# divideon/xvc

Measured on AMD Instinct MI355X. Metric: hot-path frame passes/s (TZ + sub-pel ME, MC, transform + RDOQ + dequant + inverse, deblock, pad, PSNR parts), bit-exact vs the reference's classes, higher is better.
Workload: dtype u16; 1 GPU; 1920x1080 yuv420p 30fps synthetic, QP 32, internal bitdepth 10, 16x16 CUs, TZ range 96, RDOQ (RdoQuant::QuantRdo + CoeffSignHideRdo, picture-initial CABAC contexts); cus_per_picture=8160, parallelism=3 independent picture chains in flight

## Files before the change

### xvc_amd/csrc/k_recon.h

```cpp
#ifndef XVCGPU_K_RECON_H_
#define XVCGPU_K_RECON_H_

#include <stddef.h>

#include <type_traits>

#include "dev_common.h"
#include "dev_tables.h"
#include "k_me2.h"
#include "k_tx2.h"
#include "xvcgpu_internal.h"

struct __attribute__((aligned(16))) ReconShared {
  Tx2Shared tx;
  uint16_t pred[256];
  int16_t tmp[16 * 23];
  uint16_t win[23 * 24];
};

template <bool CHROMA, int FW = 0, int FH = 0>
__device__ __forceinline__ void wave_interp_block_lds(int bd, int w_in, int h_in, int fx, int fy,
                                                      const uint16_t *ref, int rs,
                                                      uint16_t *win, int16_t *tmp,
                                                      uint16_t *dst) {
// ... 66 lines not shown
  hpass(std::true_type());
  wave_sync();
  {
    const int sh2 = 6 + (14 - bd);
    const int off2 = (8192 << 6) + (1 << (sh2 - 1));
    lane_loop<NS, 64>(lane, w * h, [&](int i) {
      const int16_t *s = tmp + i;
      int sum = 0;
#pragma unroll
      for (int k = 0; k < N; k++) sum += (int)s[k * w] * fv[k];
      dst[i] = d_clip_bd((int16_t)((sum + off2) >> sh2), smax);
    });
  }
}

template <bool RDOQ, bool FWD>
__device__ __forceinline__ void recon_from_me_kernel_body(PicView orig, PicView ref, PicView rec, const xvcgpu_me_block *blocks, const xvcgpu_me_result *results, int n_cus, int qp_y, int qp_c, int intra_pic, int ref_poc, int32_t *nnz_out, xvcgpu_cu_info *cus, const int16_t *tx_tables, const int16_t *tx_tables_t, TxTableLayout lay, const xvcgpu_rdoq_contexts *rq_ctx, const xvcgpu_rdoq_params *rq_prm, int16_t *coeffs, const uint32_t *coeff_off, FwdClassify fc) {
  constexpr int TXM = FWD ? TX_MODE_FWD : TX_MODE_FULL;
  __shared__ ReconShared s_all[4];
  union RqWave {
    RdoqShared<256> one;
    RdoqShared<64> two[2];
  };
  __shared__ RqWave rq_all[RDOQ ? 4 : 1];
  RdoqShared<256> *rq_wave = &rq_all[RDOQ ? (threadIdx.x >> 6) : 0].one;
  ReconShared &s = s_all[threadIdx.x >> 6];
  FwdClassify fcl = fc;
  if constexpr (FWD) {
    __shared__ RqProveLds pv_all[4];
    fcl.pv = (fc.cls && fc.rq_ctx && fc.rq_prm) ? &pv_all[threadIdx.x >> 6] : nullptr;
    if (fcl.pv && (threadIdx.x & 63) == 0) fcl.pv->staged_ctx = -1;
  }
  const int n = n_cus * 2;
  const int n_wg = (n + 3) / 4;
  const int wg = xcd_job_index(blockIdx.x, n_wg);
  if (wg < 0) return;
  const int job = __builtin_amdgcn_readfirstlane(wg * 4 + (int)(threadIdx.x >> 6));
  if (job >= n) return;
  const int ci = job >> 1;
  const bool chroma = (job & 1) != 0;
#ifdef XVCGPU_TRACE
  const int bi = job;
#endif
  ME2_TRACE(0);
  static_assert(offsetof(xvcgpu_me_block, y) == 2 && offsetof(xvcgpu_me_block, w) == 4 &&
                    offsetof(xvcgpu_me_block, h) == 5 && alignof(xvcgpu_me_block) >= 4,
                "xvcgpu_me_block: x, y, w, h in its first two dwords");
  const uint32_t *mbq = reinterpret_cast<const uint32_t *>(blocks + ci);
  const uint32_t mb0 = mbq[0], mb1 = mbq[1];
  const struct {
    int x, y, w, h;
  } mb = {(int16_t)(mb0 & 0xffff), (int16_t)(mb0 >> 16), (int)(mb1 & 0xff), (int)((mb1 >> 8) & 0xff)};
  const xvcgpu_me_result mr = results[ci];
  const int bd = ref.bd;
  int mx = mr.mv_x, my = mr.mv_y;
  d_clip_mv(mb.x, mb.y, ref.c[0].w, ref.c[0].h, mx, my);
  const bool cu16 = __builtin_expect(mb.w == 16 && mb.h == 16, 1);
  xvcgpu_tx_block tb;
  tb.tx_hor = XVC_TX_DEFAULT;
  tb.tx_ver = XVC_TX_DEFAULT;
  tb.dst4x4 = 0;
  tb.intra_pic = (uint8_t)intra_pic;
  if (chroma) {
    auto cjob = [&](auto exact) __attribute__((always_inline)) {
      constexpr int FS = decltype(exact)::value ? 8 : 0;
      constexpr int shift = 5;
      const int fx = mx & 31, fy = my & 31;
      const int cx = mb.x >> 1, cy = mb.y >> 1;
      const int cw = FS ? FS : mb.w >> 1, ch = FS ? FS : mb.h >> 1;
      const int lw = 31 - __clz(cw);
      tb.x = (int16_t)cx;
      tb.y = (int16_t)cy;
      tb.w = (uint8_t)cw;
      tb.h = (uint8_t)ch;
      const int g = ME2_LANE >> 5, comp = 1 + g;
      const PlaneView po = g ? orig.c[2] : orig.c[1];
      const PlaneView pc = g ? rec.c[2] : rec.c[1];
      const int i4 = (ME2_LANE & 31) * 4;
      const bool mine = i4 < cw * ch;
      U16x4 orig_pre = {{0u, 0u}};
      if (mine)
        orig_pre = *reinterpret_cast<const U16x4 *>(
            po.p + (ptrdiff_t)(cy + (i4 >> lw)) * po.stride + cx + (i4 & (cw - 1)));
#pragma unroll
      for (int c = 1; c <= 2; c++) {
        const PlaneView prf = ref.c[c];
        const uint16_t *r =
            prf.p + (ptrdiff_t)(cy + (my >> shift)) * prf.stride + cx + (mx >> shift);
        wave_interp_block_lds<true, FS, FS>(bd, cw, ch, fx, fy, r, prf.stride, s.win, s.tmp,
                                            s.pred + (c - 1) * 64);
        wave_sync();
      }
      ME2_TRACE(1);
      tb.comp = (uint8_t)comp;
      tb.qp = (int8_t)qp_c;
      if (FWD && mine)
        *reinterpret_cast<U16x4 *>(pc.p + (ptrdiff_t)(cy + (i4 >> lw)) * pc.stride + cx +
                                   (i4 & (cw - 1))) =
            *reinterpret_cast<const U16x4 *>(s.pred + g * 64 + i4);
      tx2_job<TXM, 32, RDOQ, FS, FS>(
          s.tx, tb, 3 * ci + comp, bd, po, s.pred + g * 64, cw, pc, FWD ? coeffs : nullptr,
          FWD ? coeff_off : nullptr, nnz_out, tx_tables, tx_tables_t, lay, &orig_pre, g * 128,
          reinterpret_cast<RdoqShared<64> *>(rq_wave) + g, rq_ctx, rq_prm, nullptr,
          FWD ? &fcl : nullptr);
      ME2_TRACE(8);
    };
    if (cu16) cjob(std::true_type());
    else cjob(std::false_type());
    return;
  }
  auto ljob = [&](auto exact) __attribute__((always_inline)) {
    constexpr int FS = decltype(exact)::value ? 16 : 0;
    constexpr int shift = 4;
    const int fx = mx & 15, fy = my & 15;
    const int cx = mb.x, cy = mb.y;
    const int cw = FS ? FS : mb.w, ch = FS ? FS : mb.h;
    const int lw = 31 - __clz(cw);
    tb.x = (int16_t)cx;
    tb.y = (int16_t)cy;
    tb.w = (uint8_t)cw;
    tb.h = (uint8_t)ch;
    const PlaneView prf = ref.c[0];
    const uint16_t *r = prf.p + (ptrdiff_t)(cy + (my >> shift)) * prf.stride + cx + (mx >> shift);
    U16x4 orig_pre = {{0u, 0u}};
    {
      const int i = ME2_LANE * 4;
      if (i < cw * ch) {
        const PlaneView po = orig.c[0];
        orig_pre = *reinterpret_cast<const U16x4 *>(
            po.p + (ptrdiff_t)(cy + (i >> lw)) * po.stride + cx + (i & (cw - 1)));
      }
    }
    wave_interp_block_lds<false, FS, FS>(bd, cw, ch, fx, fy, r, prf.stride, s.win, s.tmp, s.pred);
    wave_sync();
    ME2_TRACE(1);
    tb.comp = 0;
    tb.qp = (int8_t)qp_y;
    if (FWD) {
      const PlaneView pc = rec.c[0];
      lane_loop<FS * FS, 256>(ME2_LANE * 4, cw * ch, [&](int i) {
        *reinterpret_cast<U16x4 *>(pc.p + (ptrdiff_t)(cy + (i >> lw)) * pc.stride + cx +
                                   (i & (cw - 1))) = *reinterpret_cast<const U16x4 *>(s.pred + i);
      });
    }
    const int nnz = tx2_job<TXM, 64, RDOQ, FS, FS>(s.tx, tb, 3 * ci, bd, orig.c[0], s.pred, cw, rec.c[0],
                                         FWD ? coeffs : nullptr, FWD ? coeff_off : nullptr,
                                         nnz_out, tx_tables, tx_tables_t, lay, &orig_pre, 0,
                                         rq_wave, rq_ctx, rq_prm, nullptr, FWD ? &fcl : nullptr);
    ME2_TRACE(8);
    if (cus && ME2_LANE == 0) {
      xvcgpu_cu_info c;
      c.x = (uint16_t)mb.x;
      c.y = (uint16_t)mb.y;
      c.w = (uint8_t)cw;
      c.h = (uint8_t)ch;
      c.intra = 0;
      c.cbf_luma = !FWD && nnz != 0;
      c.qp_y = (int8_t)qp_y;
      c.qp_c = (int8_t)qp_c;
      c.ref_idx0 = 0;
      c.reserved = 0;
      c.ref_poc[0] = ref_poc;
      c.ref_poc[1] = -1;
      for (int k = 0; k < 4; k++) {
        c.mv[0][k][0] = mr.mv_x;
        c.mv[0][k][1] = mr.mv_y;
        c.mv[1][k][0] = 0;
        c.mv[1][k][1] = 0;
      }
      cus[ci] = c;
    }
  };
  if (cu16) ljob(std::true_type());
  else ljob(std::false_type());
}

#ifndef RECON_FWD_MIN_WAVES
#define RECON_FWD_MIN_WAVES 7
#endif
template <bool RDOQ = false, bool FWD = false>
__global__ void __launch_bounds__(256, FWD && !RDOQ ? RECON_FWD_MIN_WAVES : 1)
recon_from_me_kernel(PicView orig, PicView ref, PicView rec, const xvcgpu_me_block *blocks, const xvcgpu_me_result *results, int n_cus, int qp_y, int qp_c, int intra_pic, int ref_poc, int32_t *nnz_out, xvcgpu_cu_info *cus, const int16_t *tx_tables, const int16_t *tx_tables_t, TxTableLayout lay, const xvcgpu_rdoq_contexts *rq_ctx = nullptr, const xvcgpu_rdoq_params *rq_prm = nullptr, int16_t *coeffs = nullptr, const uint32_t *coeff_off = nullptr, FwdClassify fc = FwdClassify()) {
  recon_from_me_kernel_body<RDOQ, FWD>(orig, ref, rec, blocks, results, n_cus, qp_y, qp_c, intra_pic, ref_poc, nnz_out, cus, tx_tables, tx_tables_t, lay, rq_ctx, rq_prm, coeffs, coeff_off, fc);
}

#endif
```

### xvc_amd/csrc/k_tx2.h

```cpp
#ifndef XVCGPU_K_TX2_H_
#define XVCGPU_K_TX2_H_

#include "dev_common.h"
#include "dev_tables.h"
#include "k_me.h"
#include "k_me2.h"
#include "k_tx.h"
#include "xvcgpu_internal.h"

#define TX2_WAVES 4

typedef short tx2_v2s __attribute__((ext_vector_type(2)));

struct __attribute__((aligned(16))) Tx2Shared {
  int16_t r[256];
  int16_t t[256];
  int16_t c[256];
};

__device__ __forceinline__ int tx2_dot2(uint32_t a, uint32_t b, int acc) {
  return __builtin_amdgcn_sdot2(__builtin_bit_cast(tx2_v2s, a),
                                __builtin_bit_cast(tx2_v2s, b), acc, false);
}

template <int NJ>
__device__ __forceinline__ void tx2_load_row(const int16_t *p, uint32_t *d) {
  if (NJ == 4) {
    const uint2 v = *reinterpret_cast<const uint2 *>(p);
    d[0] = v.x; d[1] = v.y;
  } else {
#pragma unroll
    for (int q = 0; q < NJ / 8; q++) {
      const uint4 v = *reinterpret_cast<const uint4 *>(p + 8 * q);
      d[4 * q] = v.x; d[4 * q + 1] = v.y; d[4 * q + 2] = v.z; d[4 * q + 3] = v.w;
    }
  }
}

template <int NJ, int OPL, bool CLIP, int G = 64>
__device__ __forceinline__ void tx2_stage(const int16_t *A, const int16_t *B,
                                          int na, int nb, int add, int shift,
                                          int16_t *out) {
  const int lane = ME2_LANE & (G - 1);
  const int gb = nb / OPL;
  const int a = lane >> (31 - __clz(gb)), b0 = (lane & (gb - 1)) * OPL;
  if (a >= na) return;
  uint32_t ra[NJ / 2];
  tx2_load_row<NJ>(A + a * NJ, ra);
  int16_t res[OPL];
#pragma unroll
  for (int o = 0; o < OPL; o++) {
    uint32_t rb[NJ / 2];
    tx2_load_row<NJ>(B + (b0 + o) * NJ, rb);
    int acc = add;
#pragma unroll
    for (int j = 0; j < NJ / 2; j++) acc = tx2_dot2(ra[j], rb[j], acc);
    int v = acc >> shift;
    if (CLIP) v = d_clip3(v, -32768, 32767);
    res[o] = (int16_t)v;
  }
  int16_t *dst = out + a * nb + b0;
  if (OPL == 4) {
    *reinterpret_cast<uint2 *>(dst) =
        make_uint2((uint16_t)res[0] | ((uint32_t)(uint16_t)res[1] << 16),
                   (uint16_t)res[2 % OPL] | ((uint32_t)(uint16_t)res[3 % OPL] << 16));
  } else if (OPL == 2) {
    *reinterpret_cast<uint32_t *>(dst) =
        (uint16_t)res[0] | ((uint32_t)(uint16_t)res[1 % OPL] << 16);
  } else {
    dst[0] = res[0];
  }
}

template <bool CLIP, int G = 64>
__device__ __forceinline__ void tx2_stage_dispatch(int nj, const int16_t *A,
                                                   const int16_t *B, int na, int nb,
                                                   int add, int shift, int16_t *out) {
  const int total = na * nb;
  if (nj == 16) {
    if (total > 2 * G) tx2_stage<16, 4, CLIP, G>(A, B, na, nb, add, shift, out);
    else if (total > G) tx2_stage<16, 2, CLIP, G>(A, B, na, nb, add, shift, out);
    else tx2_stage<16, 1, CLIP, G>(A, B, na, nb, add, shift, out);
  } else if (nj == 8) {
    if (total > 2 * G) tx2_stage<8, 4, CLIP, G>(A, B, na, nb, add, shift, out);
    else if (total > G) tx2_stage<8, 2, CLIP, G>(A, B, na, nb, add, shift, out);
    else tx2_stage<8, 1, CLIP, G>(A, B, na, nb, add, shift, out);
  } else {
    if (total > 2 * G) tx2_stage<4, 4, CLIP, G>(A, B, na, nb, add, shift, out);
    else if (total > G) tx2_stage<4, 2, CLIP, G>(A, B, na, nb, add, shift, out);
    else tx2_stage<4, 1, CLIP, G>(A, B, na, nb, add, shift, out);
  }
}

template <int G>
__device__ __forceinline__ int tx2_group_add(int v) {
  if (G == 64) return wave_reduce_add_i32(v);
  v = dpp_group_sum<16>(v);
  return v + __shfl_xor(v, 16, 64);
}

struct FwdClassify {
  signed char *cls;
  int16_t *levels;
  int32_t *nnz;
  const xvcgpu_rdoq_contexts *rq_ctx;
  const xvcgpu_rdoq_params *rq_prm;
  RqProveLds *pv;
};

template <int MODE, int G = 64, bool RDOQ = false, int FW = 0, int FH = 0>
__device__ __forceinline__ int tx2_job(Tx2Shared &sh, const xvcgpu_tx_block &b, int bi,
                                       int bd, const PlaneView &po, const uint16_t *pred_p,
                                       int pred_stride, const PlaneView &pr,
                                       int16_t *levels, const uint32_t *level_off,
                                       int32_t *nnz_out, const int16_t *tx_tables,
                                       const int16_t *tx_tables_t,
                                       const TxTableLayout &lay,
                                       const U16x4 *orig_pre = nullptr, int soff = 0,
                                       RdoqShared<(G == 32 ? 64 : 256)> *rq = nullptr,
                                       const xvcgpu_rdoq_contexts *rq_ctx = nullptr,
                                       const xvcgpu_rdoq_params *rq_prm = nullptr,
                                       unsigned long long *dist_out = nullptr,
                                       const FwdClassify *fc = nullptr) {
  struct { int16_t *r, *t, *c; } s = {sh.r + soff, sh.t + soff, sh.c + soff};
  unsigned long long dist_acc = 0;
  auto dist4 = [&](int y, int x, const U16x4 &p, int r0, int r1, int r2, int r3) {
    const U16x4 o = *reinterpret_cast<const U16x4 *>(po.p + (ptrdiff_t)(b.y + y) * po.stride +
                                                     b.x + x);
    const int d0 = (int)(o.v[0] & 0xffff) - (int)(p.v[0] & 0xffff) - r0;
    const int d1 = (int)(o.v[0] >> 16) - (int)(p.v[0] >> 16) - r1;
    const int d2 = (int)(o.v[1] & 0xffff) - (int)(p.v[1] & 0xffff) - r2;
    const int d3 = (int)(o.v[1] >> 16) - (int)(p.v[1] >> 16) - r3;
    dist_acc += (unsigned long long)((long long)d0 * d0) + (unsigned long long)((long long)d1 * d1) +
                (unsigned long long)((long long)d2 * d2) + (unsigned long long)((long long)d3 * d3);
  };
  auto dist_finish = [&]() {
    unsigned long long v = dist_acc;
#pragma unroll
    for (int sft = 1; sft < G; sft <<= 1) v += __shfl_xor(v, sft, 64);
    if ((ME2_LANE & (G - 1)) == 0) dist_out[bi] = v >> (2 * (bd - 8));
  };
  const int lane = ME2_LANE & (G - 1);
  const int w = FW ? FW : b.w, h = FH ? FH : b.h;
  const int lw = 31 - __clz(w);
  const int lgw = lw, lgh = 31 - __clz(h);
  int16_t *lv = (levels && level_off) ? levels + level_off[bi] : nullptr;
  const int offh = tx_table_off(lay, b.tx_hor, w), offv = tx_table_off(lay, b.tx_ver, h);
  const int16_t *Mh = tx_tables + offh, *Mv = tx_tables + offv;
  const int16_t *MhT = tx_tables_t + offh, *MvT = tx_tables_t + offv;

  int qpb = b.qp + 6 * (bd - 8);
  qpb = qpb > 0 ? qpb : 0;
  const bool bias = ((lgw + lgh) & 1) != 0;
  const int tshift = 15 - bd - ((lgw + lgh) >> 1);
  const int n_el = w * h;
  constexpr int NE = FW * FH;

  int nnz;
  if (MODE != TX_MODE_INV) {
    lane_loop<NE, 4 * G>(lane * 4, n_el, [&](int i) {
      const int y = i >> lw, x = i & (w - 1);
      const U16x4 o = orig_pre ? *orig_pre
                               : *reinterpret_cast<const U16x4 *>(
                                     po.p + (ptrdiff_t)(b.y + y) * po.stride + b.x + x);
      const U16x4 p = *reinterpret_cast<const U16x4 *>(
          pred_p + (ptrdiff_t)y * pred_stride + x);
      const int d0 = (int)(o.v[0] & 0xffff) - (int)(p.v[0] & 0xffff);
      const int d1 = (int)(o.v[0] >> 16) - (int)(p.v[0] >> 16);
      const int d2 = (int)(o.v[1] & 0xffff) - (int)(p.v[1] & 0xffff);
      const int d3 = (int)(o.v[1] >> 16) - (int)(p.v[1] >> 16);
      *reinterpret_cast<uint2 *>(s.r + i) =
          make_uint2((uint32_t)(d0 & 0xffff) | ((uint32_t)d1 << 16),
                     (uint32_t)(d2 & 0xffff) | ((uint32_t)d3 << 16));
    });
    wave_sync();
    ME2_TRACE(2);
    const int shift1 = lgw + bd - 9 + (b.tx_hor == XVC_TX_DCT2_LOW ? 0 : 2);
    const int shift2 = lgh + 6 + (b.tx_ver == XVC_TX_DCT2_LOW ? 0 : 2);
    tx2_stage_dispatch<false, G>(w, Mh, s.r, w, h, 1 << (shift1 - 1), shift1, s.t);
    wave_sync();
    ME2_TRACE(3);
    tx2_stage_dispatch<false, G>(h, s.t, Mv, w, h, 1 << (shift2 - 1), shift2, s.c);
    wave_sync();
    ME2_TRACE(4);
    if (MODE == TX_MODE_FWD) {
      if (fc && fc->cls) {
        const int fq_shift = 14 + qpb / 6 + tshift + (bias ? 7 : 0);
        const int fq_scale = kFwdQuantScales[qpb % 6] * (bias ? 181 : 1);
        const long long fq_offset = 1ll << (fq_shift - 1);
        bool any = false;
        RqProveLds *pv = fc->pv;
        const int grp = ME2_LANE / G;
        if (pv) {
          if (lane == 0) {
            pv->n[grp] = 0;
            pv->fail[grp] = 0;
          }
          wave_sync();
        }
        lane_loop<NE, G>(lane, n_el, [&](int i) {
          const int a = (short)d_abs((int)s.c[i]);
          const bool nz = (short)(int)((((long long)a * fq_scale) + fq_offset) >> fq_shift) != 0;
          any |= nz;
          if (pv && nz) {
            const int slot = atomicAdd(&pv->n[grp], 1);
            if (slot < RQ_PROVE_MAX_CANDS)
              pv->xy[grp][slot] = (unsigned short)(((i & (h - 1)) << 8) | (i >> lgh));
            if (a < 0) pv->fail[grp] = 1;
          }
        });
        const unsigned long long group =
            G == 64 ? ~0ull : (((1ull << G) - 1) << (ME2_LANE & ~(G - 1)));
        bool live = (__ballot(any) & group) != 0;
        if (pv) {
          wave_sync();
          if (rq_prove_zero_lds<G>(*pv, b, bd, fc->rq_ctx, fc->rq_prm[bi], s.c, live)) live = false;
        }
        if (lane == 0) fc->cls[bi] = live ? (signed char)rq_class_of(b) : (signed char)-1;
        if (!live) {
          int16_t *z = fc->levels + level_off[bi];
          lane_loop<NE, G>(lane, n_el, [&](int i) { z[i] = 0; });
          if (lane == 0 && fc->nnz) fc->nnz[bi] = 0;
          return 0;
        }
      }
      if (lv)
        lane_loop<NE, G>(lane, n_el, [&](int i) {
          const int x = i >> lgh, k2 = i & (h - 1);
          lv[k2 * w + x] = s.c[i];
        });
      return 0;
    }
    const bool intra_pic = (b.intra_pic & XVC_TXF_INTRA_PIC) != 0;
    const bool sign_hide = !(b.intra_pic & XVC_TXF_NO_SIGN_HIDING);
    const int scan_order = (b.intra_pic >> XVC_TXF_SCAN_SHIFT) & 3;
    const int qshift = 14 + qpb / 6 + tshift + (bias ? 7 : 0);
    const int qscale = kFwdQuantScales[qpb % 6] * (bias ? 181 : 1);
    const long long qoff = (long long)((intra_pic ? 171ull : 85ull) << (qshift - 9));
    const bool use_rdoq = RDOQ && (b.intra_pic & XVC_TXF_RDOQ) != 0;
    if (RDOQ && use_rdoq) {
      const xvcgpu_rdoq_params prm = rq_prm[bi];
      const int16_t *cfp = s.c;
      int16_t *lvp = s.r;
      auto cf_at = [cfp, h](int x, int y) { return (int)cfp[x * h + y]; };
      auto lv_at = [lvp, h](int x, int y) { return lvp + x * h + y; };
      if (G == 64 && rq4_takes(64, w, h, scan_order)) {
        rq_stage_costs(&rq_ctx[prm.ctx_index], rq->ctx_bits, lane, 64);
        wave_sync();
        nnz = wave_rdoq4<64, 1>(*rq, lane, bd, w, h, b.qp, b.comp == 0, sign_hide, prm, cf_at,
                                lv_at);
      } else {
        nnz = wave_rdoq<G>(*rq, lane, bd, w, h, b.qp, b.comp == 0, scan_order, sign_hide,
                           rq_ctx[prm.ctx_index], prm, cf_at, lv_at);
      }
      wave_sync();
    }
    int local = 0;
    if (!use_rdoq) {
    for (int i = lane; i < n_el; i += G) {
      const int v = s.c[i];
      const int sign = v < 0 ? -1 : 1;
      const long long abs_coeff = d_abs(v);
      const int level = (int)(((abs_coeff * qscale) + qoff) >> qshift);
      local += level != 0;
      s.r[i] = (int16_t)d_clip3(level * sign, -32768, 32767);
      s.t[i] = (int16_t)(((abs_coeff * qscale) - ((long long)level << qshift)) >> (qshift - 8));
    }
    nnz = tx2_group_add<G>(local);
    }
    if (!use_rdoq && sign_hide && nnz > 1 && w >= 4 && h >= 4) {
      wave_sync();
      const int gw = w >> 2, gh = h >> 2;
      auto idx = [h](int x, int y) { return x * h + y; };
      const bool mine = lane < gw * gh;
      const int sx = mine ? (lane & (gw - 1)) : 0, sy = mine ? (lane >> (lgw - 2)) : 0;
      bool any = false;
      if (mine)
        for (int k = 0; k < 16; k++) any |= s.r[idx(4 * sx + (k & 3), 4 * sy + (k >> 2))] != 0;
      const int my_scan = d_sb_scan_index(scan_order, gw, gh, sx, sy);
      int last_sb = any ? my_scan : -1;
#pragma unroll
      for (int sft = 1; sft < 16; sft <<= 1) {
        const int o = __shfl_xor(last_sb, sft, 64);
// ... 73 lines not shown
      if (dist_out) dist4(y, x, p, cf, cf, cf, cf);
    });
    if (dist_out) dist_finish();
    return nnz;
  }
  {
    const int shift1 = 7 + (b.tx_ver == XVC_TX_DCT2_LOW ? 0 : 2);
    const int shift2 = 20 - bd + (b.tx_hor == XVC_TX_DCT2_LOW ? 0 : 2);
    tx2_stage_dispatch<true, G>(h, MvT, s.c, h, w, 1 << (shift1 - 1), shift1, s.r);
    wave_sync();
    tx2_stage_dispatch<true, G>(w, s.r, MhT, h, w, 1 << (shift2 - 1), shift2, s.t);
    wave_sync();
    ME2_TRACE(7);
  }
  lane_loop<NE, 4 * G>(lane * 4, n_el, [&](int i) {
    const int y = i >> lw, x = i & (w - 1);
    const U16x4 p = *reinterpret_cast<const U16x4 *>(
        pred_p + (ptrdiff_t)y * pred_stride + x);
    const uint2 rs = *reinterpret_cast<const uint2 *>(s.t + i);
    U16x4 o;
    o.v[0] = (uint32_t)d_clip3((int)(p.v[0] & 0xffff) + (int)(int16_t)(rs.x & 0xffff), 0, smax) |
             ((uint32_t)d_clip3((int)(p.v[0] >> 16) + ((int)rs.x >> 16), 0, smax) << 16);
    o.v[1] = (uint32_t)d_clip3((int)(p.v[1] & 0xffff) + (int)(int16_t)(rs.y & 0xffff), 0, smax) |
             ((uint32_t)d_clip3((int)(p.v[1] >> 16) + ((int)rs.y >> 16), 0, smax) << 16);
    *reinterpret_cast<U16x4 *>(pr.p + (ptrdiff_t)(b.y + y) * pr.stride + b.x + x) = o;
    if (dist_out)
      dist4(y, x, p, (int)(int16_t)(rs.x & 0xffff), (int)rs.x >> 16, (int)(int16_t)(rs.y & 0xffff),
            (int)rs.y >> 16);
  });
  if (dist_out) dist_finish();
  return nnz;
}

template <int MODE, bool RDOQ>
__device__ __forceinline__ void residual_wave_kernel_body(PicView orig, PicView pred, PicView rec, const xvcgpu_tx_block *blocks, int n, int16_t *levels, const uint32_t *level_off, int32_t *nnz_out, const int16_t *tx_tables, const int16_t *tx_tables_t, TxTableLayout lay, const xvcgpu_rdoq_contexts *rq_ctx, const xvcgpu_rdoq_params *rq_prm, unsigned long long *dist_out) {
  __shared__ Tx2Shared s_all[TX2_WAVES];
  __shared__ RdoqShared<256> rq_all[RDOQ ? TX2_WAVES : 1];
  Tx2Shared &s = s_all[threadIdx.x >> 6];
  const int n_wg = (n + TX2_WAVES - 1) / TX2_WAVES;
  const int wg = xcd_job_index(blockIdx.x, n_wg);
  if (wg < 0) return;
  const int bi = __builtin_amdgcn_readfirstlane(wg * TX2_WAVES + (int)(threadIdx.x >> 6));
  if (bi >= n) return;
  if (MODE == TX_MODE_INV && !dist_out && pred.c[0].p == rec.c[0].p && nnz_out[bi] == 0) return;
  const xvcgpu_tx_block b = blocks[bi];
  if (!tx_small_job(b)) return;
  const PlaneView pp = pred.c[b.comp];
  tx2_job<MODE, 64, RDOQ>(s, b, bi, pred.bd, orig.c[b.comp],
                          pp.p + (ptrdiff_t)b.y * pp.stride + b.x, pp.stride, rec.c[b.comp],
                          levels, level_off, nnz_out, tx_tables, tx_tables_t, lay, nullptr, 0,
                          &rq_all[RDOQ ? (threadIdx.x >> 6) : 0], rq_ctx, rq_prm, dist_out);
}

__global__ void __launch_bounds__(64 * TX2_WAVES)
inv_cu_pairs_kernel(PicView rec, const xvcgpu_tx_block *blocks, int n_cus, int16_t *levels,
                    const uint32_t *level_off, int32_t *nnz_out, const int16_t *tx_tables,
                    const int16_t *tx_tables_t, TxTableLayout lay) {
  const int n = 2 * n_cus;
  const int n_wg = (n + TX2_WAVES - 1) / TX2_WAVES;
  const int wg = xcd_job_index(blockIdx.x, n_wg);
  if (wg < 0) return;
  const int job = __builtin_amdgcn_readfirstlane(wg * TX2_WAVES + (int)(threadIdx.x >> 6));
  if (job >= n) return;
  const int ci = job >> 1;
  if (!(job & 1)) {
    if (nnz_out[3 * ci] == 0) return;
  } else {
    if (nnz_out[3 * ci + 1] == 0 && nnz_out[3 * ci + 2] == 0) return;
  }
  __shared__ Tx2Shared s_all[TX2_WAVES];
  Tx2Shared &s = s_all[threadIdx.x >> 6];
  if (!(job & 1)) {
    const int bi = 3 * ci;
    const xvcgpu_tx_block b = blocks[bi];
    if (!tx_small_job(b)) return;
    const PlaneView pc = rec.c[0];
    const uint16_t *at = pc.p + (ptrdiff_t)b.y * pc.stride + b.x;
    if (__builtin_expect(b.w == 16 && b.h == 16, 1))
      tx2_job<TX_MODE_INV, 64, false, 16, 16>(s, b, bi, rec.bd, pc, at, pc.stride, pc, levels,
                                              level_off, nnz_out, tx_tables, tx_tables_t, lay);
    else
      tx2_job<TX_MODE_INV, 64, false>(s, b, bi, rec.bd, pc, at, pc.stride, pc, levels, level_off,
                                      nnz_out, tx_tables, tx_tables_t, lay);
    return;
  }
  const int g = ME2_LANE >> 5, bi = 3 * ci + 1 + g;
  const xvcgpu_tx_block b = blocks[bi];
  if (!tx_small_job(b) || b.w * b.h > 64) return;
  const PlaneView pc = g ? rec.c[2] : rec.c[1];
  const uint16_t *at = pc.p + (ptrdiff_t)b.y * pc.stride + b.x;
  if (__builtin_expect(b.w == 8 && b.h == 8, 1))
    tx2_job<TX_MODE_INV, 32, false, 8, 8>(s, b, bi, rec.bd, pc, at, pc.stride, pc, levels,
                                          level_off, nnz_out, tx_tables, tx_tables_t, lay,
                                          nullptr, g * 128);
  else
    tx2_job<TX_MODE_INV, 32, false>(s, b, bi, rec.bd, pc, at, pc.stride, pc, levels, level_off,
                                    nnz_out, tx_tables, tx_tables_t, lay, nullptr, g * 128);
}

template <int MODE, bool RDOQ = false>
__global__ void __launch_bounds__(64 * TX2_WAVES)
residual_wave_kernel(PicView orig, PicView pred, PicView rec, const xvcgpu_tx_block *blocks, int n, int16_t *levels, const uint32_t *level_off, int32_t *nnz_out, const int16_t *tx_tables, const int16_t *tx_tables_t, TxTableLayout lay, const xvcgpu_rdoq_contexts *rq_ctx = nullptr, const xvcgpu_rdoq_params *rq_prm = nullptr, unsigned long long *dist_out = nullptr) {
  residual_wave_kernel_body<MODE, RDOQ>(orig, pred, rec, blocks, n, levels, level_off, nnz_out, tx_tables, tx_tables_t, lay, rq_ctx, rq_prm, dist_out);
}

template <int MODE, bool RDOQ>
__device__ __forceinline__ void
residual_cu_body(const PicView &orig, const PicView &pred, const PicView &rec, const xvcgpu_tx_block *blocks, int n,
                   int16_t *levels, const uint32_t *level_off, int32_t *nnz_out,
                   const int16_t *tx_tables, const int16_t *tx_tables_t, TxTableLayout lay,
                   const xvcgpu_rdoq_contexts *rq_ctx, const xvcgpu_rdoq_params *rq_prm,
                   const xvcgpu_block_pos *src_pos, const xvcgpu_eval_cand *ecands, int n_head,
                   uint64_t *eout, int strength) {
  struct Big {
    TxShared s;
    RdoqShared<RDOQ ? 1024 : 4> rq;
  };
  struct Small {
    Tx2Shared s;
    RdoqShared<256> rq;
  };
  constexpr size_t kBytes = sizeof(Big) > sizeof(Small) ? sizeof(Big) : sizeof(Small);
  __shared__ __attribute__((aligned(16))) unsigned char raw[kBytes];
  const int idx = blockIdx.x;
  auto price = [&](int c) {
    const xvcgpu_eval_cand cd = ecands[c];
    const PlaneView pa = orig.c[cd.comp], pb = cd.versus ? rec.c[cd.comp] : pred.c[cd.comp];
    const uint16_t *a = cd.orig_at ? pa.p + (ptrdiff_t)cd.oy * pa.stride + cd.ox
                                   : pa.p + (ptrdiff_t)cd.y * pa.stride + cd.x;
    const uint16_t *bq = pb.p + (ptrdiff_t)cd.y * pb.stride + cd.x;
    const uint64_t dist = wave_compare(cd.metric, orig.bd, cd.qp, strength, cd.w, cd.h, a,
                                       pa.stride, bq, pb.stride);
    if ((threadIdx.x & 63) == 0) eout[c] = (uint64_t)((double)dist * cd.weight);
  };
  if (idx >= n) {
    if (ecands && idx - n < n_head && threadIdx.x < 64) price(idx - n);
    return;
  }
  if (MODE == TX_MODE_INV && pred.c[0].p == rec.c[0].p && nnz_out[idx] == 0) return;
  const xvcgpu_tx_block b = blocks[idx];
  const PlaneView pp = pred.c[b.comp];
  PicView orig_v = orig;
  const uint16_t *pred_p = pp.p + (ptrdiff_t)b.y * pp.stride + b.x;
  if (src_pos) {
// ... 43 lines not shown
```

### xvc_amd/csrc/xvcgpu.hip

```cpp
#include <hip/hip_runtime.h>
#include <stdlib.h>
#include <stdio.h>
#include <string.h>

#include <algorithm>
#include <new>
#include <vector>

#include "k_deblock.h"
#include "k_tail.h"
#include "k_me.h"
#include "k_me2.h"
#include "k_me_plan.h"
#include "k_metric.h"
#include "k_misc.h"
#include "k_pad.h"
#include "k_tx.h"
#include "k_tx2.h"
#include "k_recon.h"
#include "k_bipred.h"
#include "k_stats.h"
#include "k_output.h"
#include "k_intra.h"
#include "k_affine_me.h"
// ... 1538 lines not shown
  ctx->rdoq_classified_proved = prove;
  const int n_wg = (2 * n + 3) / 4;
  hipLaunchKernelGGL((recon_from_me_kernel<false, true>), dim3((n_wg + 7) / 8 * 8), dim3(256), 0,
                     ctx->stream, orig->v, ref->v, pred->v, d_blocks, d_results, n, qp_y, qp_c, 0,
                     ref_poc, nullptr, d_cus, ctx->d_tx_tables, ctx->d_tx_tables_t,
                     xvcgpu_tx_layout(), nullptr, nullptr, d_coeffs, d_coeff_offsets, fc);
  CHECK_LAUNCH(ctx, "fwd_from_me_classify");
  return XVCGPU_OK;
}

xvcgpu_status xvcgpu_fwd_transform_batch(xvcgpu_ctx *ctx,
                                         const xvcgpu_picture *orig,
                                         const xvcgpu_picture *pred,
                                         const xvcgpu_tx_block *d_blocks, int n,
                                         int16_t *d_coeffs,
                                         const uint32_t *d_coeff_offsets) {
  if (!ctx || !orig || !pred || n < 0 ||
      (n && (!d_blocks || !d_coeffs || !d_coeff_offsets)))
    return XVCGPU_INVALID_ARGUMENT;
  if (n == 0) return XVCGPU_OK;
  launch_residual<TX_MODE_FWD>(ctx, orig->v, pred->v, pred->v, d_blocks, n, d_coeffs,
                               d_coeff_offsets, (int32_t *)nullptr);
  CHECK_LAUNCH(ctx, "fwd_transform_batch");
  return XVCGPU_OK;
}

xvcgpu_status xvcgpu_inv_transform_batch(xvcgpu_ctx *ctx,
                                         const xvcgpu_picture *pred,
                                         xvcgpu_picture *rec,
                                         const xvcgpu_tx_block *d_blocks, int n,
                                         const int16_t *d_levels,
                                         const uint32_t *d_level_offsets,
                                         const int32_t *d_nnz) {
  if (!ctx || !pred || !rec || n < 0 ||
      (n && (!d_blocks || !d_levels || !d_level_offsets || !d_nnz)))
    return XVCGPU_INVALID_ARGUMENT;
  if (n == 0) return XVCGPU_OK;
  launch_residual<TX_MODE_INV>(ctx, pred->v, pred->v, rec->v, d_blocks, n,
                               const_cast<int16_t *>(d_levels), d_level_offsets,
                               const_cast<int32_t *>(d_nnz));
  CHECK_LAUNCH(ctx, "inv_transform_batch");
  return XVCGPU_OK;
}

xvcgpu_status xvcgpu_inv_transform_cu_order(xvcgpu_ctx *ctx, xvcgpu_picture *rec,
                                            const xvcgpu_tx_block *d_blocks, int n_cus,
                                            const int16_t *d_levels,
                                            const uint32_t *d_level_offsets,
                                            const int32_t *d_nnz) {
  if (!ctx || !rec || n_cus < 0 ||
      (n_cus && (!d_blocks || !d_levels || !d_level_offsets || !d_nnz)))
    return XVCGPU_INVALID_ARGUMENT;
  if (n_cus == 0) return XVCGPU_OK;
  const int n_wg = (2 * n_cus + TX2_WAVES - 1) / TX2_WAVES;
  hipLaunchKernelGGL(inv_cu_pairs_kernel, dim3((n_wg + 7) / 8 * 8), dim3(64 * TX2_WAVES), 0,
                     ctx->stream, rec->v, d_blocks, n_cus, const_cast<int16_t *>(d_levels),
                     d_level_offsets, const_cast<int32_t *>(d_nnz), ctx->d_tx_tables,
                     ctx->d_tx_tables_t, xvcgpu_tx_layout());
  CHECK_LAUNCH(ctx, "inv_transform_cu_order");
  return XVCGPU_OK;
}

xvcgpu_status xvcgpu_inv_transform_dist_batch(xvcgpu_ctx *ctx, const xvcgpu_picture *orig,
                                              const xvcgpu_picture *pred, xvcgpu_picture *rec,
                                              const xvcgpu_tx_block *d_blocks, int n,
                                              const int16_t *d_levels,
                                              const uint32_t *d_level_offsets,
                                              const int32_t *d_nnz, uint64_t *d_dist) {
  if (!ctx || !orig || !pred || !rec || n < 0 ||
      (n && (!d_blocks || !d_levels || !d_level_offsets || !d_nnz || !d_dist)))
    return XVCGPU_INVALID_ARGUMENT;
  if (orig->w != pred->w || orig->h != pred->h || orig->bd != pred->bd)
    return fail(ctx, XVCGPU_INVALID_ARGUMENT, "picture mismatch");
  if (n == 0) return XVCGPU_OK;
  launch_residual<TX_MODE_INV>(ctx, orig->v, pred->v, rec->v, d_blocks, n,
                               const_cast<int16_t *>(d_levels), d_level_offsets,
                               const_cast<int32_t *>(d_nnz),
                               reinterpret_cast<unsigned long long *>(d_dist));
  CHECK_LAUNCH(ctx, "inv_transform_dist_batch");
  return XVCGPU_OK;
}

xvcgpu_status xvcgpu_tx_eval_batch(xvcgpu_ctx *ctx, const xvcgpu_tx_eval_job *d_jobs, int n,
                                   const xvcgpu_tx_eval_alt *d_alts,
                                   xvcgpu_tx_eval_result *d_out) {
  if (!ctx || n < 0 || (n && (!d_jobs || !d_alts || !d_out))) return XVCGPU_INVALID_ARGUMENT;
  if (n == 0) return XVCGPU_OK;
  HIP_TRY(ctx, hipSetDevice(ctx->device));
  hipLaunchKernelGGL(tx_eval_kernel, dim3((n + 255) / 256), dim3(256), 0, ctx->stream, d_jobs, n,
                     d_alts, d_out);
  CHECK_LAUNCH(ctx, "tx_eval_batch");
  return XVCGPU_OK;
}

xvcgpu_status xvcgpu_root_cbf_batch(xvcgpu_ctx *ctx, const xvcgpu_root_cbf_job *d_jobs, int n,
                                    xvcgpu_root_cbf_result *d_out) {
  if (!ctx || n < 0 || (n && (!d_jobs || !d_out))) return XVCGPU_INVALID_ARGUMENT;
  if (n == 0) return XVCGPU_OK;
  HIP_TRY(ctx, hipSetDevice(ctx->device));
  hipLaunchKernelGGL(root_cbf_kernel, dim3((n + 255) / 256), dim3(256), 0, ctx->stream, d_jobs, n,
                     d_out);
  CHECK_LAUNCH(ctx, "root_cbf_batch");
  return XVCGPU_OK;
}

static xvcgpu_status deblock_rows_masked(xvcgpu_ctx *ctx, xvcgpu_picture *rec,
// ... 1655 lines not shown
```

Before: 8962 frame passes/s.

## Specialize exact DCT2 inverse path and stage transform matrices in LDS

```diff
diff --git a/xvc_amd/csrc/k_recon.h b/xvc_amd/csrc/k_recon.h
--- a/xvc_amd/csrc/k_recon.h
+++ b/xvc_amd/csrc/k_recon.h
@@ -142,6 +142,24 @@
     int x, y, w, h;
   } mb = {(int16_t)(mb0 & 0xffff), (int16_t)(mb0 >> 16), (int)(mb1 & 0xff), (int)((mb1 >> 8) & 0xff)};
   const xvcgpu_me_result mr = results[ci];
+  Tx2FwdPre pre = {}, pre_v = {};
+  if constexpr (FWD) {
+    const int pbi = 3 * ci + (chroma ? 1 : 0);
+    pre.lo = coeff_off[pbi];
+    if (chroma) pre_v.lo = coeff_off[pbi + 1];
+    if (fc.cls && fc.rq_ctx && fc.rq_prm) {
+      constexpr int NW = sizeof(RqParamWords) / 4;
+      const uint32_t *pw = reinterpret_cast<const uint32_t *>(fc.rq_prm + pbi);
+#pragma unroll
+      for (int k = 0; k < NW; k++) pre.prm.v[k] = pw[k];
+      if (chroma) {
+#pragma unroll
+        for (int k = 0; k < NW; k++) pre_v.prm.v[k] = pw[NW + k];
+      }
+    }
+    tx2_to_scalar(pre);
+    if (chroma) tx2_to_scalar(pre_v);
+  }
   const int bd = ref.bd;
   int mx = mr.mv_x, my = mr.mv_y;
   d_clip_mv(mb.x, mb.y, ref.c[0].w, ref.c[0].h, mx, my);
@@ -172,6 +190,12 @@
       if (mine)
         orig_pre = *reinterpret_cast<const U16x4 *>(
             po.p + (ptrdiff_t)(cy + (i4 >> lw)) * po.stride + cx + (i4 & (cw - 1)));
+      constexpr bool MLDS = FWD && FS > 0;
+      uint32_t mword = 0;
+      if (MLDS && ME2_LANE < 32)
+        mword = *reinterpret_cast<const uint32_t *>(tx_tables + tx_table_off(lay, XVC_TX_DCT2, 8) +
+                                                    2 * ME2_LANE);
+      int16_t *m_lds = reinterpret_cast<int16_t *>(s.win);
 #pragma unroll
       for (int c = 1; c <= 2; c++) {
         const PlaneView prf = ref.c[c];
@@ -184,15 +208,17 @@
       ME2_TRACE(1);
       tb.comp = (uint8_t)comp;
       tb.qp = (int8_t)qp_c;
+      if (MLDS && ME2_LANE < 32) *reinterpret_cast<uint32_t *>(m_lds + 2 * ME2_LANE) = mword;
+      const Tx2FwdPre pre_g = g ? pre_v : pre;
       if (FWD && mine)
         *reinterpret_cast<U16x4 *>(pc.p + (ptrdiff_t)(cy + (i4 >> lw)) * pc.stride + cx +
                                    (i4 & (cw - 1))) =
             *reinterpret_cast<const U16x4 *>(s.pred + g * 64 + i4);
-      tx2_job<TXM, 32, RDOQ, FS, FS>(
+      tx2_job<TXM, 32, RDOQ, FS, FS, MLDS>(
           s.tx, tb, 3 * ci + comp, bd, po, s.pred + g * 64, cw, pc, FWD ? coeffs : nullptr,
           FWD ? coeff_off : nullptr, nnz_out, tx_tables, tx_tables_t, lay, &orig_pre, g * 128,
           reinterpret_cast<RdoqShared<64> *>(rq_wave) + g, rq_ctx, rq_prm, nullptr,
-          FWD ? &fcl : nullptr);
+          FWD ? &fcl : nullptr, m_lds, FWD ? &pre_g : nullptr);
       ME2_TRACE(8);
     };
     if (cu16) cjob(std::true_type());
@@ -221,11 +247,18 @@
             po.p + (ptrdiff_t)(cy + (i >> lw)) * po.stride + cx + (i & (cw - 1)));
       }
     }
+    constexpr bool MLDS = FWD && FS > 0;
+    uint2 mword = make_uint2(0u, 0u);
+    if (MLDS)
+      mword = *reinterpret_cast<const uint2 *>(tx_tables + tx_table_off(lay, XVC_TX_DCT2, 16) +
+                                               4 * ME2_LANE);
+    int16_t *m_lds = reinterpret_cast<int16_t *>(s.win);
     wave_interp_block_lds<false, FS, FS>(bd, cw, ch, fx, fy, r, prf.stride, s.win, s.tmp, s.pred);
     wave_sync();
     ME2_TRACE(1);
     tb.comp = 0;
     tb.qp = (int8_t)qp_y;
+    if (MLDS) *reinterpret_cast<uint2 *>(m_lds + 4 * ME2_LANE) = mword;
     if (FWD) {
       const PlaneView pc = rec.c[0];
       lane_loop<FS * FS, 256>(ME2_LANE * 4, cw * ch, [&](int i) {
@@ -233,10 +266,10 @@
                                    (i & (cw - 1))) = *reinterpret_cast<const U16x4 *>(s.pred + i);
       });
     }
-    const int nnz = tx2_job<TXM, 64, RDOQ, FS, FS>(s.tx, tb, 3 * ci, bd, orig.c[0], s.pred, cw, rec.c[0],
-                                         FWD ? coeffs : nullptr, FWD ? coeff_off : nullptr,
-                                         nnz_out, tx_tables, tx_tables_t, lay, &orig_pre, 0,
-                                         rq_wave, rq_ctx, rq_prm, nullptr, FWD ? &fcl : nullptr);
+    const int nnz = tx2_job<TXM, 64, RDOQ, FS, FS, MLDS>(
+        s.tx, tb, 3 * ci, bd, orig.c[0], s.pred, cw, rec.c[0], FWD ? coeffs : nullptr,
+        FWD ? coeff_off : nullptr, nnz_out, tx_tables, tx_tables_t, lay, &orig_pre, 0, rq_wave,
+        rq_ctx, rq_prm, nullptr, FWD ? &fcl : nullptr, m_lds, FWD ? &pre : nullptr);
     ME2_TRACE(8);
     if (cus && ME2_LANE == 0) {
       xvcgpu_cu_info c;
diff --git a/xvc_amd/csrc/k_tx2.h b/xvc_amd/csrc/k_tx2.h
--- a/xvc_amd/csrc/k_tx2.h
+++ b/xvc_amd/csrc/k_tx2.h
@@ -1,5 +1,9 @@
 #ifndef XVCGPU_K_TX2_H_
 #define XVCGPU_K_TX2_H_
+
+#include <stddef.h>
+
+#include <type_traits>
 
 #include "dev_common.h"
 #include "dev_tables.h"
@@ -34,6 +38,24 @@
       const uint4 v = *reinterpret_cast<const uint4 *>(p + 8 * q);
       d[4 * q] = v.x; d[4 * q + 1] = v.y; d[4 * q + 2] = v.z; d[4 * q + 3] = v.w;
     }
+  }
+}
+
+template <int NJ, int OPL, bool CLIP>
+__device__ __forceinline__ void tx2_stage_lane(const int16_t *a_row, const int16_t *b_rows,
+                                               int add, int shift, int16_t *res) {
+  uint32_t ra[NJ / 2];
+  tx2_load_row<NJ>(a_row, ra);
+#pragma unroll
+  for (int o = 0; o < OPL; o++) {
+    uint32_t rb[NJ / 2];
+    tx2_load_row<NJ>(b_rows + o * NJ, rb);
+    int acc = add;
+#pragma unroll
+    for (int j = 0; j < NJ / 2; j++) acc = tx2_dot2(ra[j], rb[j], acc);
+    int v = acc >> shift;
+    if (CLIP) v = d_clip3(v, -32768, 32767);
+    res[o] = (int16_t)v;
   }
 }
 
@@ -108,7 +130,27 @@
   RqProveLds *pv;
 };
 
-template <int MODE, int G = 64, bool RDOQ = false, int FW = 0, int FH = 0>
+struct __attribute__((packed, aligned(2))) U16x2 {
+  uint32_t v[1];
+};
+
+struct RqParamWords {
+  uint32_t v[sizeof(xvcgpu_rdoq_params) / 4];
+};
+static_assert(sizeof(RqParamWords) == sizeof(xvcgpu_rdoq_params) && alignof(xvcgpu_rdoq_params) >= 4,
+              "xvcgpu_rdoq_params: whole dwords");
+struct Tx2FwdPre {
+  uint32_t lo;
+  RqParamWords prm;
+};
+__device__ __forceinline__ void tx2_to_scalar(Tx2FwdPre &p) {
+  p.lo = (uint32_t)__builtin_amdgcn_readfirstlane((int)p.lo);
+#pragma unroll
+  for (unsigned k = 0; k < sizeof(p.prm.v) / 4; k++)
+    p.prm.v[k] = (uint32_t)__builtin_amdgcn_readfirstlane((int)p.prm.v[k]);
+}
+
+template <int MODE, int G = 64, bool RDOQ = false, int FW = 0, int FH = 0, bool MLDS = false>
 __device__ __forceinline__ int tx2_job(Tx2Shared &sh, const xvcgpu_tx_block &b, int bi,
                                        int bd, const PlaneView &po, const uint16_t *pred_p,
                                        int pred_stride, const PlaneView &pr,
@@ -121,7 +163,10 @@
                                        const xvcgpu_rdoq_contexts *rq_ctx = nullptr,
                                        const xvcgpu_rdoq_params *rq_prm = nullptr,
                                        unsigned long long *dist_out = nullptr,
-                                       const FwdClassify *fc = nullptr) {
+                                       const FwdClassify *fc = nullptr,
+                                       const int16_t *m_lds = nullptr,
+                                       const Tx2FwdPre *pre = nullptr) {
+  static_assert(!MLDS || (MODE == TX_MODE_FWD && FW > 0 && FW == FH), "MLDS: forward, square, exact");
   struct { int16_t *r, *t, *c; } s = {sh.r + soff, sh.t + soff, sh.c + soff};
   unsigned long long dist_acc = 0;
   auto dist4 = [&](int y, int x, const U16x4 &p, int r0, int r1, int r2, int r3) {
@@ -144,10 +189,13 @@
   const int w = FW ? FW : b.w, h = FH ? FH : b.h;
   const int lw = 31 - __clz(w);
   const int lgw = lw, lgh = 31 - __clz(h);
-  int16_t *lv = (levels && level_off) ? levels + level_off[bi] : nullptr;
+  int16_t *lv = (levels && level_off) ? levels + (pre ? pre->lo : level_off[bi]) : nullptr;
   const int offh = tx_table_off(lay, b.tx_hor, w), offv = tx_table_off(lay, b.tx_ver, h);
-  const int16_t *Mh = tx_tables + offh, *Mv = tx_tables + offv;
+  const int16_t *Mh = MLDS ? m_lds : tx_tables + offh, *Mv = MLDS ? m_lds : tx_tables + offv;
   const int16_t *MhT = tx_tables_t + offh, *MvT = tx_tables_t + offv;
+  constexpr bool ROWS = FW > 0 && FW == FH && G == 4 * FW;
+  constexpr int NL = ROWS ? FW / 4 : 2;
+  using RowWords = typename std::conditional<NL == 4, U16x4, U16x2>::type;
 
   int qpb = b.qp + 6 * (bd - 8);
   qpb = qpb > 0 ? qpb : 0;
@@ -214,21 +262,39 @@
         bool live = (__ballot(any) & group) != 0;
         if (pv) {
           wave_sync();
-          if (rq_prove_zero_lds<G>(*pv, b, bd, fc->rq_ctx, fc->rq_prm[bi], s.c, live)) live = false;
+          if (rq_prove_zero_lds<G>(*pv, b, bd, fc->rq_ctx, pre ? __builtin_bit_cast(xvcgpu_rdoq_params, pre->prm) : fc->rq_prm[bi],
+                                   s.c, live))
+            live = false;
         }
         if (lane == 0) fc->cls[bi] = live ? (signed char)rq_class_of(b) : (signed char)-1;
         if (!live) {
-          int16_t *z = fc->levels + level_off[bi];
-          lane_loop<NE, G>(lane, n_el, [&](int i) { z[i] = 0; });
+          int16_t *z = fc->levels + (pre ? pre->lo : level_off[bi]);
+          if constexpr (ROWS) {
+            const RowWords zero = {};
+            *reinterpret_cast<RowWords *>(z + lane * NL) = zero;
+          } else {
+            lane_loop<NE, G>(lane, n_el, [&](int i) { z[i] = 0; });
+          }
           if (lane == 0 && fc->nnz) fc->nnz[bi] = 0;
           return 0;
         }
       }
-      if (lv)
-        lane_loop<NE, G>(lane, n_el, [&](int i) {
-          const int x = i >> lgh, k2 = i & (h - 1);
-          lv[k2 * w + x] = s.c[i];
-        });
+      if (lv) {
+        if constexpr (ROWS) {
+          const int k2 = lane >> 2, x0 = (lane & 3) * NL;
+          RowWords o;
+#pragma unroll
+          for (int j = 0; j < NL / 2; j++)
+            o.v[j] = (uint32_t)(uint16_t)s.c[(x0 + 2 * j) * FW + k2] |
+                     ((uint32_t)(uint16_t)s.c[(x0 + 2 * j + 1) * FW + k2] << 16);
+          *reinterpret_cast<RowWords *>(lv + lane * NL) = o;
+        } else {
+          lane_loop<NE, G>(lane, n_el, [&](int i) {
+            const int x = i >> lgh, k2 = i & (h - 1);
+            lv[k2 * w + x] = s.c[i];
+          });
+        }
+      }
       return 0;
     }
     const bool intra_pic = (b.intra_pic & XVC_TXF_INTRA_PIC) != 0;
@@ -408,10 +474,118 @@
                           &rq_all[RDOQ ? (threadIdx.x >> 6) : 0], rq_ctx, rq_prm, dist_out);
 }
 
-__global__ void __launch_bounds__(64 * TX2_WAVES)
-inv_cu_pairs_kernel(PicView rec, const xvcgpu_tx_block *blocks, int n_cus, int16_t *levels,
-                    const uint32_t *level_off, int32_t *nnz_out, const int16_t *tx_tables,
+struct TxBlockWords {
+  uint32_t v[3];
+};
+static_assert(sizeof(xvcgpu_tx_block) == sizeof(TxBlockWords) &&
+                  offsetof(xvcgpu_tx_block, y) == 2 && offsetof(xvcgpu_tx_block, w) == 4 &&
+                  offsetof(xvcgpu_tx_block, h) == 5 && offsetof(xvcgpu_tx_block, tx_hor) == 7 &&
+                  offsetof(xvcgpu_tx_block, tx_ver) == 8 && offsetof(xvcgpu_tx_block, qp) == 10,
+              "xvcgpu_tx_block: three dwords, x y | w h comp tx_hor | tx_ver dst4x4 qp flags");
+
+__device__ __forceinline__ void tx2_pin(int &nnz, TxBlockWords &q, uint32_t &lo) {
+  asm("" : "+s"(nnz), "+s"(q.v[0]), "+s"(q.v[1]), "+s"(q.v[2]), "+s"(lo));
+}
+__device__ __forceinline__ void tx2_pin(int &nnz_u, int &nnz_v, TxBlockWords &q_u,
+                                        TxBlockWords &q_v, uint32_t &lo_u, uint32_t &lo_v) {
+  asm("" : "+s"(nnz_u), "+s"(nnz_v), "+s"(q_u.v[0]), "+s"(q_u.v[1]), "+s"(q_u.v[2]),
+           "+s"(q_v.v[0]), "+s"(q_v.v[1]), "+s"(q_v.v[2]), "+s"(lo_u), "+s"(lo_v));
+}
+
+__device__ __forceinline__ bool tx2_is_dct2(int type) {
+  return type == XVC_TX_DEFAULT || type == XVC_TX_DCT2;
+}
+
+template <int FS>
+__device__ __forceinline__ bool tx2_exact_dct2(const TxBlockWords &q) {
+  return (q.v[1] & 0xffff) == (uint32_t)(FS | (FS << 8)) && tx2_is_dct2(q.v[1] >> 24) &&
+         tx2_is_dct2(q.v[2] & 0xff);
+}
+
+__device__ __forceinline__ void tx2_dequant_square(int qp, int bd, int lg, int &scale, int &shift) {
+  int qpb = qp + 6 * (bd - 8);
+  qpb = qpb > 0 ? qpb : 0;
+  shift = 6 - (15 - bd - lg);
+  constexpr unsigned long long kScales = 0x484039332d28ull;
+  scale = (int)((kScales >> (8 * (qpb % 6))) & 0xff) << (qpb / 6);
+}
+
+template <int G, int FS>
+__device__ __forceinline__ void tx2_inv_exact(int16_t *sc, int16_t *sr, int16_t *m,
+                                              const int16_t *mt, bool active, int nnz, int bx,
+                                              int by, int scale, int shift, int bd,
+                                              const PlaneView &pc, const int16_t *lv) {
+  static_assert((G == 64 && FS == 16) || (G == 32 && FS == 8), "a quarter row per lane");
+  constexpr int NL = FS / 4;
+  using Words = typename std::conditional<NL == 4, U16x4, U16x2>::type;
+  const int lane = ME2_LANE & (G - 1);
+  const int row = lane >> 2, col = (lane & 3) * NL;
+  uint16_t *at = pc.p + (ptrdiff_t)(by + row) * pc.stride + bx + col;
+  Words lw = {}, pw = {};
+  if (active) {
+    lw = *reinterpret_cast<const Words *>(lv + lane * NL);
+    pw = *reinterpret_cast<const Words *>(at);
+  }
+  if (FS == 16) {
+    *reinterpret_cast<uint2 *>(m + 4 * ME2_LANE) =
+        *reinterpret_cast<const uint2 *>(mt + 4 * ME2_LANE);
+  } else if (ME2_LANE < 32) {
+    *reinterpret_cast<uint32_t *>(m + 2 * ME2_LANE) =
+        *reinterpret_cast<const uint32_t *>(mt + 2 * ME2_LANE);
+  }
+  if (!active) return;
+  int q[NL];
+#pragma unroll
+  for (int j = 0; j < NL; j++) {
+    const int level = (int16_t)(lw.v[j >> 1] >> (16 * (j & 1)));
+    const int prod = level * scale;
+    int cf;
+    if (shift > 0) cf = (prod + (1 << (shift - 1))) >> shift;
+    else cf = (int)((unsigned)prod << -shift);
+    q[j] = d_clip3(cf, -32768, 32767);
+  }
+  const int smax = (1 << bd) - 1;
+  auto add_clip_store = [&](const int *r) {
+    Words o;
+#pragma unroll
+    for (int j = 0; j < NL / 2; j++)
+      o.v[j] = (uint32_t)d_clip3((int)(pw.v[j] & 0xffff) + r[2 * j], 0, smax) |
+               ((uint32_t)d_clip3((int)(pw.v[j] >> 16) + r[2 * j + 1], 0, smax) << 16);
+    *reinterpret_cast<Words *>(at) = o;
+  };
+  const uint32_t first = (lw.v[0] & 0xffff) | ((uint32_t)q[0] << 16);
+  const uint32_t first_g = G == 64 ? (uint32_t)__builtin_amdgcn_readfirstlane((int)first)
+                                   : (uint32_t)__shfl((int)first, ME2_LANE & 32, 64);
+  if (nnz == 1 && (first_g & 0xffff) != 0) {
+    const int sh = 14 - bd, add = 1 << (sh - 1);
+    const int c0 = (int)first_g >> 16;
+    const int cf = (int16_t)((((c0 + 1) >> 1) + add) >> sh);
+    int r[NL];
+#pragma unroll
+    for (int j = 0; j < NL; j++) r[j] = cf;
+    add_clip_store(r);
+    return;
+  }
+#pragma unroll
+  for (int j = 0; j < NL; j++) sc[(col + j) * FS + row] = (int16_t)q[j];
+  wave_sync();
+  const int shift1 = 7 + 2, shift2 = 20 - bd + 2;
+  tx2_stage<FS, NL, true, G>(m, sc, FS, FS, 1 << (shift1 - 1), shift1, sr);
+  wave_sync();
+  int16_t res[NL];
+  tx2_stage_lane<FS, NL, true>(sr + row * FS, m + col * FS, 1 << (shift2 - 1), shift2, res);
+  int r[NL];
+#pragma unroll
+  for (int j = 0; j < NL; j++) r[j] = res[j];
+  add_clip_store(r);
+}
+
+__global__ void __launch_bounds__(64 * TX2_WAVES, 8)
+inv_cu_pairs_kernel(PicView rec, const xvcgpu_tx_block *__restrict__ blocks, int n_cus,
+                    int16_t *levels, const uint32_t *__restrict__ level_off,
+                    const int32_t *__restrict__ nnz_in, const int16_t *tx_tables,
                     const int16_t *tx_tables_t, TxTableLayout lay) {
+  int32_t *nnz_out = const_cast<int32_t *>(nnz_in);
   const int n = 2 * n_cus;
   const int n_wg = (n + TX2_WAVES - 1) / TX2_WAVES;
   const int wg = xcd_job_index(blockIdx.x, n_wg);
@@ -419,20 +593,30 @@
   const int job = __builtin_amdgcn_readfirstlane(wg * TX2_WAVES + (int)(threadIdx.x >> 6));
   if (job >= n) return;
   const int ci = job >> 1;
-  if (!(job & 1)) {
-    if (nnz_out[3 * ci] == 0) return;
-  } else {
-    if (nnz_out[3 * ci + 1] == 0 && nnz_out[3 * ci + 2] == 0) return;
-  }
   __shared__ Tx2Shared s_all[TX2_WAVES];
+  __shared__ __attribute__((aligned(16))) int16_t m_all[TX2_WAVES][256];
   Tx2Shared &s = s_all[threadIdx.x >> 6];
+  int16_t *m = m_all[threadIdx.x >> 6];
+  const TxBlockWords *headers = reinterpret_cast<const TxBlockWords *>(blocks);
   if (!(job & 1)) {
     const int bi = 3 * ci;
-    const xvcgpu_tx_block b = blocks[bi];
+    int nnz = nnz_in[bi];
+    TxBlockWords q = headers[bi];
+    uint32_t lo = level_off[bi];
+    tx2_pin(nnz, q, lo);
+    if (nnz == 0) return;
+    const xvcgpu_tx_block b = __builtin_bit_cast(xvcgpu_tx_block, q);
+    const PlaneView pc = rec.c[0];
+    if (__builtin_expect(tx2_exact_dct2<16>(q), 1)) {
+      int scale, shift;
+      tx2_dequant_square(b.qp, rec.bd, 4, scale, shift);
+      tx2_inv_exact<64, 16>(s.c, s.r, m, tx_tables_t + tx_table_off(lay, XVC_TX_DCT2, 16), true,
+                            nnz, b.x, b.y, scale, shift, rec.bd, pc, levels + lo);
+      return;
+    }
     if (!tx_small_job(b)) return;
-    const PlaneView pc = rec.c[0];
     const uint16_t *at = pc.p + (ptrdiff_t)b.y * pc.stride + b.x;
-    if (__builtin_expect(b.w == 16 && b.h == 16, 1))
+    if (b.w == 16 && b.h == 16)
       tx2_job<TX_MODE_INV, 64, false, 16, 16>(s, b, bi, rec.bd, pc, at, pc.stride, pc, levels,
                                               level_off, nnz_out, tx_tables, tx_tables_t, lay);
     else
@@ -440,12 +624,32 @@
                                       nnz_out, tx_tables, tx_tables_t, lay);
     return;
   }
-  const int g = ME2_LANE >> 5, bi = 3 * ci + 1 + g;
-  const xvcgpu_tx_block b = blocks[bi];
+  const int bi_u = 3 * ci + 1;
+  int nnz_u = nnz_in[bi_u], nnz_v = nnz_in[bi_u + 1];
+  TxBlockWords q_u = headers[bi_u], q_v = headers[bi_u + 1];
+  uint32_t lo_u = level_off[bi_u], lo_v = level_off[bi_u + 1];
+  tx2_pin(nnz_u, nnz_v, q_u, q_v, lo_u, lo_v);
+  if (nnz_u == 0 && nnz_v == 0) return;
+  const int g = ME2_LANE >> 5, bi = bi_u + g;
+  TxBlockWords q;
+#pragma unroll
+  for (int k = 0; k < 3; k++) q.v[k] = g ? q_v.v[k] : q_u.v[k];
+  const xvcgpu_tx_block b = __builtin_bit_cast(xvcgpu_tx_block, q);
+  const PlaneView pc = g ? rec.c[2] : rec.c[1];
+  if (__builtin_expect(tx2_exact_dct2<8>(q_u) && tx2_exact_dct2<8>(q_v), 1)) {
+    int scale_u, scale_v, shift_u, shift_v;
+    tx2_dequant_square((int8_t)(q_u.v[2] >> 16), rec.bd, 3, scale_u, shift_u);
+    tx2_dequant_square((int8_t)(q_v.v[2] >> 16), rec.bd, 3, scale_v, shift_v);
+    const int nnz = g ? nnz_v : nnz_u;
+    tx2_inv_exact<32, 8>(s.c + g * 128, s.r + g * 128, m,
+                         tx_tables_t + tx_table_off(lay, XVC_TX_DCT2, 8), nnz != 0, nnz, b.x, b.y,
+                         g ? scale_v : scale_u, g ? shift_v : shift_u, rec.bd, pc,
+                         levels + (g ? lo_v : lo_u));
+    return;
+  }
   if (!tx_small_job(b) || b.w * b.h > 64) return;
-  const PlaneView pc = g ? rec.c[2] : rec.c[1];
   const uint16_t *at = pc.p + (ptrdiff_t)b.y * pc.stride + b.x;
-  if (__builtin_expect(b.w == 8 && b.h == 8, 1))
+  if (b.w == 8 && b.h == 8)
     tx2_job<TX_MODE_INV, 32, false, 8, 8>(s, b, bi, rec.bd, pc, at, pc.stride, pc, levels,
                                           level_off, nnz_out, tx_tables, tx_tables_t, lay,
                                           nullptr, g * 128);
diff --git a/xvc_amd/csrc/xvcgpu.hip b/xvc_amd/csrc/xvcgpu.hip
--- a/xvc_amd/csrc/xvcgpu.hip
+++ b/xvc_amd/csrc/xvcgpu.hip
@@ -1614,6 +1614,7 @@
       (n_cus && (!d_blocks || !d_levels || !d_level_offsets || !d_nnz)))
     return XVCGPU_INVALID_ARGUMENT;
   if (n_cus == 0) return XVCGPU_OK;
+  if ((uintptr_t)d_blocks & 3) return fail(ctx, XVCGPU_INVALID_ARGUMENT, "d_blocks: 4-byte alignment");
   const int n_wg = (2 * n_cus + TX2_WAVES - 1) / TX2_WAVES;
   hipLaunchKernelGGL(inv_cu_pairs_kernel, dim3((n_wg + 7) / 8 * 8), dim3(64 * TX2_WAVES), 0,
                      ctx->stream, rec->v, d_blocks, n_cus, const_cast<int16_t *>(d_levels),
```

Measured after the change: 9251 frame passes/s (median of 5 runs). 1.03x the previous value.
